# microsoft/maro

Hardware: AMD Instinct MI355X
Metric: env-steps/sec (decision events/sec), CIM global_trade.22p (higher is better)
Workload: dtype int32+f64

## Files before the change

maro_amd/csrc/cim_device.h:

```cpp
#pragma once
#include <math.h>
#include <stdint.h>

#include "cim_params.h"

#ifdef MRX_SPECIALIZED
#define KD(f) (MRXC_##f)
#define OD(f) (MRXC_obs_##f)
#define ODA(f, i) (MRXC_obs_##f(i))
#else
#define KD(f) (K.f)
#define OD(f) (O.f)
#define ODA(f, i) (O.f[i])
#endif

namespace cim {

#ifndef MRX_PROFILE_PHASES
struct Prof {
  MRX_DEV void mark(int) {}
  MRX_DEV void mark(int, long long) {}
  MRX_DEV void flush() {}
};
#endif
// ... 2133 lines not shown
#ifdef MRX_LEAN2
    const Tabs& T = L.tab;
    const int a_vs0 = wave::readlane(Z.s.vs0, v), a_Lr = a_vs0 & 63, a_rb = (int)((unsigned)a_vs0 >> 12), a_cb = wave::readlane(Z.s.vs2, v);
    const int a_lr = wave::lane() < a_Lr ? wave::lane() : 0;
    const int a_rp = T.route_port[a_rb + a_lr], a_rc = T.route_cidx[a_rb + a_lr], a_per = V_PERIOD(v);
#endif
    const int pe_v = FP(PA_EMPTY, p), ve_v = FV(VA_EMPTY, v), rs_v = FV(VA_REMAINING_SPACE, v), tc_v = FP(PA_TRANSFER_COST, p);
    const int pe = U(pe_v), ve = U(ve_v), rs = U(rs_v), tc = U(tc_v);
    int npe, nve;
    if (ty == 1) {
      if (q > ve) { c.status |= 1; continue; }
      npe = pe + q; nve = ve - q;
    } else {
      if (q > (pe < rs ? pe : rs)) { c.status |= 1; continue; }
      npe = pe - q; nve = ve + q;
    }
    FP(PA_EMPTY, p) = npe;
    FV(VA_EMPTY, v) = nve;
    FV(VA_REMAINING_SPACE, v) = rs - (nve - ve);
    c.opnum += q;
    FP(PA_TRANSFER_COST, p) = f_bits((float)((double)bits_f(tc) + (double)q));
    {
#ifdef MRX_LEAN2
      const uint64_t hit = wave::ballot(wave::lane() < a_Lr && a_rp == p);
      const int cc = hit ? a_cb + wave::readlane(a_rc, __builtin_ctzll(hit)) : -1;
      if (cc >= 0) { const int pl = U(L.frame[KD(f_plans) + cc]); L.frame[KD(f_plans) + cc] = pl + U(a_per); }
#else
      const int cc = plan_cell(L, v, p);
      if (cc >= 0) { const int pl = U(L.frame[KD(f_plans) + cc]); L.frame[KD(f_plans) + cc] = pl + U(V_PERIOD(v)); }
#endif
      else c.status |= 32;
    }
  }
  c.pend = consume_decisions(K, c.pend, L.priv[PH_CUR_VESSEL], c.n_answered);
  wave::sync();
}

template <bool PG, bool OBS>
MRX_DEV StepEnd body_run(const CimParams& K, const CimObs& O, int env, Lds& L, const StepIO& io, StepCtx& c, StepOut& out, Prof& prof, RingRegs& rr, Lean& Z) {
  const int lane = wave::lane();
  const int P = KD(P), V = KD(V);
  StepEnd end = {true, false, false};
  int t = c.t;
  bool fresh = c.fresh, finished = false;
  uint64_t pend = c.pend;
  int dec_v = -1;
  for (;;) {
    if (pend) {
      dec_v = __builtin_ctzll(pend);
      break;
    }
    if (!fresh) {
      if ((t + 1) % KD(resolution) == 0) {
        if (lane < P) FP(PA_ACC_FULFILLMENT, lane) = FP(PA_ACC_BOOKING, lane) - FP(PA_ACC_SHORTAGE, lane);
        wave::sync();
        take_snapshot(K, O, env, L, (t - KD(start_tick)) / KD(resolution));
        wave::sync();
        if (lane < P) { FP(PA_SHORTAGE, lane) = 0; FP(PA_BOOKING, lane) = 0; FP(PA_FULFILLMENT, lane) = 0; FP(PA_TRANSFER_COST, lane) = 0; }
        wave::sync();
      }
      if (t + 1 == KD(T)) {
        if ((t + 1) % KD(resolution) != 0) take_snapshot(K, O, env, L, (t - KD(start_tick)) / KD(resolution));
        finished = true;
        break;
      }
      t += 1;
    }
    prof.mark(PF_POST_STEP);
    fresh = false;
#ifdef MRX_LEAN2
    pend = run_tick_lean(K, env, L, t, c.pf, c.idx_buf, c.status, prof, end.buf_dirty, rr, Z);
#else
    pend = run_tick<PG>(K, env, L, t, c.pf, c.idx_ord, c.idx_buf, c.status, prof, end.ord_dirty, end.buf_dirty, rr);
#endif
    if (!pend && t + 1 < KD(T)) {
#ifdef MRX_LEAN2
      tick_prefetch_lean(K, env, L, t + 1, c.pf, Z);
#else
      tick_prefetch<PG>(K, env, L, t + 1, c.pf);
#endif
      tick_prefetch_land(c.pf);
    }
  }

  if (MRX_UNALIGNED_FRAMES && !finished) {
    const int fi0 = (t - KD(start_tick)) / KD(resolution), lo = KD(start_tick) + fi0 * KD(resolution);
    if (t > lo + (KD(resolution) - 1 - lo % KD(resolution))) {
      wave::sync();
      take_snapshot(K, O, env, L, fi0);
      wave::sync();
    }
  }
  long long acc_b = 0, acc_s = 0;
  if (lane < P) { acc_b = FP(PA_ACC_BOOKING, lane); acc_s = FP(PA_ACC_SHORTAGE, lane); }
  acc_b = wave::reduce_add(acc_b);
  acc_s = wave::reduce_add(acc_s);
  const int fi = (t - KD(start_tick)) / KD(resolution);
  out.kind = 1;
  if (KD(decision_mode) != 0) {
    int32_t* dec_out = io.dec_out;
    const uint64_t pm = finished ? 0ull : pend;
    const bool mine = lane < V && ((pm >> lane) & 1ull);
    if (mine) {
      const int r = __builtin_popcountll(pm & ((1ull << lane) - 1ull));
      const int v = lane, p = FV(VA_LOC_PORT_IDX, v);
      const int pe = FP(PA_EMPTY, p), rs = FV(VA_REMAINING_SPACE, v);
      int32_t* d = dec_out + 8 * r;
      d[0] = t; d[1] = p; d[2] = v; d[3] = pe < rs ? pe : rs; d[4] = FV(VA_EMPTY, v); d[5] = FV(VA_EARLY_DISCHARGE, v);
      d[6] = fi; d[7] = 1;
    }
    const int cnt = __builtin_popcountll(pm);
    if (lane < V && lane >= cnt) {
      int32_t* d = dec_out + 8 * lane;
      for (int j = 0; j < 8; j++) d[j] = 0;
      if (lane == 0) { d[0] = t; d[6] = fi; }
    }
  } else if (!finished) {
    {
      const int v = dec_v, p = FV(VA_LOC_PORT_IDX, v);
      const int pe = FP(PA_EMPTY, p), rs = FV(VA_REMAINING_SPACE, v);
      out.dec[0] = t; out.dec[1] = p; out.dec[2] = v;
      out.dec[3] = pe < rs ? pe : rs;
      out.dec[4] = FV(VA_EMPTY, v);
      out.dec[5] = FV(VA_EARLY_DISCHARGE, v);
      out.dec[6] = fi; out.dec[7] = 1;
    }
    if constexpr (OBS) {
      out.obs_on = true;
      const int tot = P * OD(np), npd = OD(np) > 0 ? OD(np) : 1;
#pragma unroll
      for (int j = 0; j < 8; j++) {
        const int i = lane + 64 * j;
        out.obs[j] = 0.0;
        if (i < tot) {
          const int p = i / npd, a = i - p * npd;
          const int attr = (int)((OD(pa_packed) >> (4 * a)) & 15u);
          out.obs[j] = port_attr_value(attr, FP(attr, p));
        }
      }
#pragma unroll
      for (int a = 0; a < 8; a++) out.vobs[a] = a < OD(nv) ? (double)FV(ODA(va, a), dec_v) : 0.0;
    }
  } else {
    out.dec[0] = t; out.dec[1] = 0; out.dec[2] = 0; out.dec[3] = 0; out.dec[4] = 0; out.dec[5] = 0;
    out.dec[6] = fi; out.dec[7] = 0;
  }
  out.met[0] = acc_b; out.met[1] = acc_s; out.met[2] = c.opnum;
  out.done = finished ? 1 : 0;
  out.tick = t;
  out.status = c.status;
  out.hint = (KD(decision_mode) == 0 && !MRX_UNALIGNED_FRAMES && (finished || (pend & ~(1ull << (dec_v & 63))))) ? 0 : 1;
  bool long_next = false;
  if (KD(start_tick) == 0 && !finished) {
#ifdef MRX_LEAN2
    const bool soon = lane < V && (vr_park(Z.w) ? Z.w.next : Z.w.evt) <= t + 1;
#else
    const bool soon = lane < V && (FV(VA_IS_PARKING, lane) ? V_NEXT(lane) : V_EVT(lane)) <= t + 1;
#endif
    long_next = wave::ballot(soon) == 0ull;
  }
  if (long_next && out.hint) out.hint = 2;
  if (lane == 0) {
    L.priv[PH_TICK] = t;
    L.priv[PH_FLAGS] = finished ? FL_FINISHED : (long_next ? FL_LONG : 0);
    L.priv[PH_PEND_LO] = (int32_t)(uint32_t)(pend & 0xffffffffull);
    L.priv[PH_PEND_HI] = (int32_t)(uint32_t)(pend >> 32);
    L.priv[PH_CUR_VESSEL] = dec_v;
    L.priv[PH_OPNUM_LO] = (int32_t)(uint32_t)((unsigned long long)c.opnum & 0xffffffffull);
    L.priv[PH_OPNUM_HI] = (int32_t)(c.opnum >> 32);
    L.priv[PH_IDX_ORDER] = c.idx_ord;
    L.priv[PH_IDX_BUFFER] = c.idx_buf;
    L.priv[PH_ACCB_LO] = (int32_t)(uint32_t)((unsigned long long)acc_b & 0xffffffffull); L.priv[PH_ACCB_HI] = (int32_t)(acc_b >> 32);
    L.priv[PH_ACCS_LO] = (int32_t)(uint32_t)((unsigned long long)acc_s & 0xffffffffull); L.priv[PH_ACCS_HI] = (int32_t)(acc_s >> 32);
  }
  wave::sync();
  prof.mark(PF_OUTPUT);
  return end;
}

template <bool OBS>
MRX_DEV void body_emit(const CimParams& K, const CimObs& O, int env, const StepIO& io, const StepOut& out, long long agent_seed) {
  const int lane = wave::lane();
  if (out.kind == 0) return;
  if (out.kind == 2) {
    if (lane < 8) io.dec_out[lane] = lane == 7 ? -1 : 0;
    if (lane < 3) io.met_out[lane] = 0;
    if (lane == 0) { *io.done_out = 1; if (O.agent_mode) agent_none(O, env); }
    return;
  }
  if (O.agent_mode && KD(decision_mode) == 0 && lane == 0) {
    if (out.dec[7] == 1 && !out.done) agent_answer(K, O, env, agent_seed, out.dec[0], out.dec[1], out.dec[2], out.dec[3], out.dec[4]);
    else agent_none(O, env);
  }
  if (KD(decision_mode) == 0) {
    if (lane == 0) {
#pragma unroll
      for (int j = 0; j < 8; j++) io.dec_out[j] = out.dec[j];
    }
    if constexpr (OBS) {
      if (out.obs_on) {
        const int tot = KD(P) * OD(np);
        double* op = O.ports + (size_t)env * tot;
#pragma unroll
        for (int j = 0; j < 8; j++) {
          const int i = lane + 64 * j;
          if (i < tot) op[i] = out.obs[j];
        }
#pragma unroll
        for (int a = 0; a < 8; a++)
          if (a < OD(nv) && lane == 0) O.vessel[(size_t)env * OD(nv) + a] = out.vobs[a];
      }
    }
  }
  if (lane == 0) {
    io.met_out[0] = out.met[0]; io.met_out[1] = out.met[1]; io.met_out[2] = out.met[2];
    *io.done_out = (uint8_t)out.done;
    K.tick[env] = out.tick;
    K.hint[env] = (uint8_t)out.hint;
    if (out.status) wave::global_or(&K.status[env], out.status);
  }
}

template <bool PG, bool OBS>
MRX_DEV StepEnd full_body(const CimParams& K, const CimObs& O, int env, Lds& L, const StepIO& io, int a0v, int a0p, int a0q, int a0t, Prof& prof, RingRegs& rr, Lean& Z) {
  StepCtx c;
  StepOut out;
  c.a0v = a0v; c.a0p = a0p; c.a0q = a0q; c.a0t = a0t;
  c.n_act = io.n_act; c.n_answered = io.n_answered;
  StepEnd end = {false, false, false};
  const long long agent_seed = O.agent_mode ? K.seed[env] : 0;
  if (body_open<PG>(K, env, L, c, out, Z)) {
    prof.mark(PF_LOAD);
    body_act(K, L, io.actions, c, Z);
    prof.mark(PF_ACTION);
    tick_prefetch_land(c.pf);
    prof.mark(PF_MT_LOAD);
    end = body_run<PG, OBS>(K, O, env, L, io, c, out, prof, rr, Z);
  }
  body_emit<OBS>(K, O, env, io, out, agent_seed);
  return end;
}

enum { PATH_PROBE = 0,
       PATH_FAST = 1,
       PATH_FULL = 2 };

template <bool PG, bool OBS>
MRX_DEV void step_env(const CimParams& K, const CimObs& O, int env, int32_t* lds, const StepIO& io, int path, int32_t* lds_ctab = nullptr) {
  Lds L = make_lds(K, lds);
  Prof prof;
  if (KD(decision_mode) == 0 && path != PATH_FULL) {
    FastRows rows;
    fast_rows_request<OBS>(K, O, env, rows);
    int hint = 0;
    if (path == PATH_PROBE) hint = K.hint[env];
    int f0v = 0, f0p = 0, f0q = 0, f0t = 0;
    if (io.actions) { f0v = io.actions[0]; f0p = io.actions[1]; f0q = io.actions[2]; f0t = io.actions[3]; }
    if (!U(hint) && fast_step<OBS>(K, O, env, rows, io.n_act > KD(max_actions) ? KD(max_actions) : io.n_act, f0v, f0p, f0q, f0t, io.dec_out,
                                   io.met_out, io.done_out)) {
#ifdef MRX_PROFILE_FAST_PATH
      prof.mark(13); prof.mark(14, 1);
      prof.flush();
#endif
      return;
    }
    prof.mark(12);
  }
  state_load_async<PG>(K, L, env);
  stage_tables(K, L, lds_ctab ? lds_ctab : lds + KD(l_ctab));
  RingRegs rr;
  ring_load(K, env, rr);
  Lean Z;
#ifdef MRX_LEAN2
  lean_stat_load(K, Z.s);
#endif
  int a0v = 0, a0p = 0, a0q = 0, a0t = 0;
  if (io.actions) { a0v = io.actions[0]; a0p = io.actions[1]; a0q = io.actions[2]; a0t = io.actions[3]; }
  wave::lds_dma_wait();
  const StepEnd e = full_body<PG, OBS>(K, O, env, L, io, a0v, a0p, a0q, a0t, prof, rr, Z);
  if (e.store) { state_store<PG>(K, L, env, e); ring_store(K, env, rr); }
  prof.mark(PF_STORE);
  prof.flush();
}

template <bool OBS>
MRX_DEV void fast_lanes_env(const CimParams& K, const CimObs& O, const StepBatch& B, const uint8_t* mask, int env) {
  if (env >= K.n_envs || (mask && !mask[env]) || K.hint[env]) return;
  const StepIO io = step_io(K, B, env);
  const int n_act = io.n_act > KD(max_actions) ? KD(max_actions) : io.n_act;
  if (KD(decision_mode) == 0 && fast_step_lane<OBS>(K, O, env, io.actions, n_act, io.dec_out, io.met_out, io.done_out)) return;
  K.order[wave::global_add(&K.sched[0], 1)] = env | MRX_ORDER_TICK;
}

template <bool PG, bool OBS>
MRX_DEV void step_loop(const CimParams& K, const CimObs& O, int32_t* lds, int w, int W, const StepBatch& B) {
  const int n_tick = U(wave::ld_uniform_v(K.sched + 0));
  for (int i = w; i < n_tick; i += W) {
    const int env = U(wave::ld_uniform_v(K.order + i)) & (MRX_ORDER_TICK - 1);
    step_env<PG, OBS>(K, O, env, lds, step_io(K, B, env), PATH_FULL);
    wave::sync();
  }
}

MRX_DEV int attr_slots(const CimParams& K, int node_type, int a) {
  if (node_type == 0) return 1;
  if (node_type == 1) {
    if (a == VA_PAST_STOP_LIST || a == VA_PAST_STOP_TICK_LIST) return KD(past_n);
    if (a == VA_FUTURE_STOP_LIST || a == VA_FUTURE_STOP_TICK_LIST) return KD(future_n);
    return 1;
  }
  return a == MA_FULL_ON_PORTS ? KD(P) * KD(P) : KD(V) * KD(P);
}

MRX_DEV int frame_word(const CimParams& K, int node_type, int a, int node, int s) {
  if (node_type == 0) return KD(f_ports) + a * KD(P) + node;
  if (node_type == 1) return KD(f_vessels) + a * KD(V) + node;
  if (a == MA_FULL_ON_PORTS) {
    const int k = K.pair_dense[s];
    return k < 0 ? -1 : KD(f_fop) + k;
  }
  const int c = K.cidx_dense[s];
  if (c < 0) return -1;
  return (a == MA_FULL_ON_VESSELS ? KD(f_fov) : KD(f_plans)) + c;
}

MRX_DEV int stop_list_value(const CimParams& K, int env, const int32_t* frame, int a, int v, int s) {
  const int Lr = K.v_route_len[v], rb = K.v_route_base[v], start = K.v_start[v];
  const uint32_t* srow = K.stops + ((size_t)env * KD(V) + v) * KD(SMAX);
  if (a == VA_PAST_STOP_LIST || a == VA_PAST_STOP_TICK_LIST) {
    const int j = frame[KD(f_vessels) + VA_NEXT_LOC_IDX * KD(V) + v] - KD(past_n) + s;
    if (j < 0) return -1;
    if (a == VA_PAST_STOP_LIST) return K.route_port[rb + (start + j) % Lr];
    if (j == 0) {
      const int32_t* hdr = K.priv + (size_t)env * KD(PW);
      const uint64_t zm = ((uint64_t)(uint32_t)hdr[PH_ZOMBIE_HI] << 32) | (uint32_t)hdr[PH_ZOMBIE_LO];
      if (!((zm >> v) & 1ull)) return 0;
    }
    return stop_arrival(srow[j < KD(SMAX) ? j : KD(SMAX) - 1]);
  }
  const int k = frame[KD(f_vessels) + VA_LAST_LOC_IDX * KD(V) + v];
  int tick = k == 0 ? 0 : stop_arrival(srow[k < KD(SMAX) ? k : KD(SMAX) - 1]);
  int x = (start + k) % Lr;
  const int lo = K.leg_off[v];
  for (int i = 0; i <= s; i++) {
    tick += K.leg_time[lo + x];
    x = (x + 1 == Lr) ? 0 : x + 1;
  }
  return a == VA_FUTURE_STOP_LIST ? K.route_port[rb + x] : tick;
}

MRX_DEV const int32_t* frame_of(const CimParams& K, int env, int fi) {
  const int s = (fi < 0 ? 0 : fi) % KD(S);
  const int32_t* hdr = K.priv + (size_t)env * KD(PW);
  const int flags = hdr[PH_FLAGS], tick = hdr[PH_TICK], held = K.ring_fi[(size_t)env * KD(S) + s];
  const bool paused = (flags & (FL_FRESH | FL_FINISHED)) == 0;
  const int cur_fi = (tick - KD(start_tick)) / KD(resolution);
  const int32_t* frame = nullptr;
  if (held == fi) frame = K.ring + ((size_t)env * KD(S) + s) * KD(FW);
  if (paused && s == cur_fi % KD(S)) frame = fi == cur_fi ? K.live + (size_t)env * KD(FW) : nullptr;
  return fi < 0 ? nullptr : frame;
}

MRX_DEV double query_elem(const CimParams& K, int node_type, const int32_t* ticks, int nt, int ticks_per_env,
                          const int32_t* nodes, int nn, int nodes_per_env, const int32_t* attrs, int na, long long row, int col) {
  const int ni = (int)(row % nn);
  const int ti = (int)((row / nn) % nt);
  const int env = (int)(row / ((long long)nn * nt));
  const int fi = ticks[(size_t)env * ticks_per_env + ti];
  const int32_t* frame = frame_of(K, env, fi);
  if (!frame) return 0.0;
  int a = 0, slot = col;
  for (int i = 0; i < na; i++) {
    const int ns = attr_slots(K, node_type, attrs[i]);
    if (slot < ns) { a = attrs[i]; break; }
    slot -= ns;
  }
  const int node = nodes[(size_t)env * nodes_per_env + ni];
  const int n_nodes = node_type == 0 ? KD(P) : node_type == 1 ? KD(V) : 1;
  if (node < 0 || node >= n_nodes) return 0.0;
  if (node_type == 1 && a >= VA_PAST_STOP_LIST) return (double)stop_list_value(K, env, frame, a, node, slot);
  const int w = frame_word(K, node_type, a, node, slot);
  if (w < 0) return a == MA_VESSEL_PLANS ? -1.0 : 0.0;
  const int32_t raw = frame[w];
  return (node_type == 0 && a == PA_TRANSFER_COST) ? (double)bits_f(raw) : (double)raw;
}

#undef FP
#undef FV
#undef FOPK
#undef FOVC
#undef PLANC
#undef V_EVT
#undef V_NEXT
#undef V_POS
#undef V_KRL
#undef V_PERIOD
#undef U
#undef RING_FULL
#undef RING_EMPTY

}
```

maro_amd/csrc/cim_step_kernels.h:

```cpp
extern "C" __global__ void __launch_bounds__(64)
mrx_k_cim_reset(CimParams K, const long long* __restrict__ seed_cmd, const uint8_t* __restrict__ mask, long long default_cmd) {
  extern __shared__ __attribute__((aligned(16))) int32_t lds[];
  const int env = blockIdx.x;
  if (mask && !mask[env]) return;
  cim::reset_env(K, env, lds, seed_cmd ? seed_cmd[env] : default_cmd);
}

extern "C" __global__ void __launch_bounds__(64)
mrx_k_cim_order_table(CimParams K, const long long* __restrict__ seed_cmd, const uint8_t* __restrict__ mask, long long default_cmd) {
  extern __shared__ __attribute__((aligned(16))) int32_t lds[];
  const int env = blockIdx.x;
  if (mask && !mask[env]) return;
  if ((seed_cmd ? seed_cmd[env] : default_cmd) == -1) return;
  cim::gen_order_table(K, env, lds);
}

#ifndef MRX_STEP_WAVES
#define MRX_STEP_WAVES 2
#endif
#ifdef MRX_SPECIALIZED
#define MRX_WG_WAVES MRXC_wg_waves
#else
#define MRX_WG_WAVES 1
#endif
#define MRX_STEP_KERNEL(NAME, PG, OBS, WAVES)                                                                            \
  extern "C" __global__ void __launch_bounds__(64 * MRX_WG_WAVES, WAVES)                                                 \
  NAME(CimParams K, CimObs O, cim::StepBatch B, const uint8_t* __restrict__ mask, int sorted) {                          \
    extern __shared__ __attribute__((aligned(16))) int32_t lds[];                                                       \
    const int w = MRX_WG_WAVES > 1 ? __builtin_amdgcn_readfirstlane((int)(threadIdx.x >> 6)) : 0;                        \
    const int slot = (int)blockIdx.x * MRX_WG_WAVES + w;                                                                \
    if (MRX_WG_WAVES > 1 && slot >= K.n_envs) return;                                                                   \
    int env = slot, path = cim::PATH_PROBE;                                                                             \
    if (sorted) {                                                                                                       \
      if (sorted == 2 && slot >= K.sched[0]) return;   \
      const int e = K.order[slot];                                                                                      \
      if (e < 0) return;                                                                                                \
      env = e & (MRX_ORDER_TICK - 1);                                                                                   \
      path = (e & MRX_ORDER_TICK) ? cim::PATH_FULL : cim::PATH_FAST;                                                    \
    } else if (mask && !mask[env]) {                                                                                    \
      return;                                                                                                           \
    }                                                                                                                   \
    cim::step_env<PG, OBS>(K, O, env, lds + w * KD(l_ctab), cim::step_io(K, B, env), path,                               \
                           lds + MRX_WG_WAVES * KD(l_ctab));                                                            \
  }
#ifdef MRX_SPECIALIZED
#define MRX_WANT(PG, OBS) ((PG) == (MRXC_pregen != 0) && (OBS) == ((MRXC_obs_np | MRXC_obs_nv) != 0))
#else
#define MRX_WANT(PG, OBS) 1
#endif
#define MRX_SPLIT_KERNELS(SUFFIX, PG, OBS, WAVES)                                                                       \
  extern "C" __global__ void __launch_bounds__(64)                                                                      \
  mrx_k_cim_fast_lanes##SUFFIX(CimParams K, CimObs O, cim::StepBatch B, const uint8_t* __restrict__ mask) {               \
    cim::fast_lanes_env<OBS>(K, O, B, mask, (int)(blockIdx.x * 64 + threadIdx.x));                                      \
  }                                                                                                                     \
  extern "C" __global__ void __launch_bounds__(64, WAVES)                                                               \
  mrx_k_cim_step_loop##SUFFIX(CimParams K, CimObs O, cim::StepBatch B) {                                                 \
    extern __shared__ __attribute__((aligned(16))) int32_t lds[];                                                       \
    cim::step_loop<PG, OBS>(K, O, lds, (int)blockIdx.x, (int)gridDim.x, B);                                             \
  }
#if MRX_WANT(0, 0)
MRX_STEP_KERNEL(mrx_k_cim_step, false, false, MRX_STEP_WAVES)
MRX_SPLIT_KERNELS(, false, false, MRX_STEP_WAVES)
#endif
#if MRX_WANT(0, 1)
MRX_STEP_KERNEL(mrx_k_cim_step_obs, false, true, MRX_STEP_WAVES)
MRX_SPLIT_KERNELS(_obs, false, true, MRX_STEP_WAVES)
#endif
#if MRX_WANT(1, 0)
MRX_STEP_KERNEL(mrx_k_cim_step_tab, true, false, MRX_STEP_WAVES)
MRX_SPLIT_KERNELS(_tab, true, false, MRX_STEP_WAVES)
#endif
#if MRX_WANT(1, 1)
MRX_STEP_KERNEL(mrx_k_cim_step_tab_obs, true, true, MRX_STEP_WAVES)
MRX_SPLIT_KERNELS(_tab_obs, true, true, MRX_STEP_WAVES)
#endif
#undef MRX_WANT
#undef MRX_STEP_KERNEL
#undef MRX_SPLIT_KERNELS
```

Measured before the change: 153.7 million.

## Add lane-parallel fast-path slots with ballot-driven full-step fallback in step kernel

Moves the per-slot dispatch into a new step_slot helper. Under MRX_LANE_WAVES with sorted==1, waves beyond the tick count each run the fast step for 64 environments at once, one per lane. Any lanes the fast path refuses are collected by ballot and then run serially through the full step_env on the same wave. This is meant to avoid a separate fast-lanes kernel launch and the one-env-per-wave cost of the fast path, at the price of serialised redo work and more branch complexity. Without the macro the behaviour is the same as before.

```diff
diff --git a/maro_amd/csrc/cim_device.h b/maro_amd/csrc/cim_device.h
--- a/maro_amd/csrc/cim_device.h
+++ b/maro_amd/csrc/cim_device.h
@@ -2459,6 +2459,70 @@
   }
 }
 
+template <bool PG, bool OBS>
+MRX_DEV void step_slot(const CimParams& K, const CimObs& O, const StepBatch& B, const uint8_t* mask, int sorted, int slot, int32_t* lds,
+                       int32_t* lds_ctab) {
+  int env = slot, path = PATH_PROBE;
+#ifdef MRX_LANE_WAVES
+  uint64_t redo = 0;
+  int redo_base = 0;
+  if (sorted == 1) {
+    const int e = K.order[slot], n_tick = K.sched[0], n_all = K.sched[1];
+    path = PATH_FULL;
+    if (e >= 0 && (e & MRX_ORDER_TICK)) {
+      env = e & (MRX_ORDER_TICK - 1);
+    } else {
+      const int w = slot - n_tick, n_fast = n_all - n_tick;
+      if (w < 0 || w >= ((n_fast + 63) >> 6)) return;
+      redo_base = n_tick + 64 * w;
+#ifdef MRX_PROFILE_FAST_PATH
+      Prof prof;
+#endif
+      const int i = redo_base + wave::lane();
+      bool refused = false;
+      if (i < n_all) {
+        const int lenv = K.order[i];
+        const StepIO io = step_io(K, B, lenv);
+        const int n_act = io.n_act > KD(max_actions) ? KD(max_actions) : io.n_act;
+        refused = !(KD(decision_mode) == 0 && fast_step_lane<OBS>(K, O, lenv, io.actions, n_act, io.dec_out, io.met_out, io.done_out));
+      }
+      redo = wave::ballot(refused);
+#ifdef MRX_PROFILE_FAST_PATH
+      prof.mark(13); prof.mark(14, __builtin_popcountll(wave::ballot(i < n_all) & ~redo));
+      prof.flush();
+#endif
+      if (!redo) return;
+      env = K.order[redo_base + __builtin_ctzll(redo)];
+      redo &= redo - 1;
+    }
+  } else
+#endif
+  if (sorted) {
+    if (sorted == 2 && slot >= K.sched[0]) return;
+    const int e = K.order[slot];
+    if (e < 0) return;
+    env = e & (MRX_ORDER_TICK - 1);
+    path = (e & MRX_ORDER_TICK) ? PATH_FULL : PATH_FAST;
+  } else if (mask && !mask[env]) {
+    return;
+  }
+#ifdef MRX_LANE_WAVES
+  for (;;) {
+    int z = 0;
+#if defined(__HIP_DEVICE_COMPILE__)
+    asm volatile("" : "+s"(z));
+#endif
+    step_env<PG, OBS>(K, O, env, lds + z, step_io(K, B, env), path, lds_ctab + z);
+    if (!redo) break;
+    wave::sync();
+    env = K.order[redo_base + __builtin_ctzll(redo)];
+    redo &= redo - 1;
+  }
+#else
+  step_env<PG, OBS>(K, O, env, lds, step_io(K, B, env), path, lds_ctab);
+#endif
+}
+
 MRX_DEV int attr_slots(const CimParams& K, int node_type, int a) {
   if (node_type == 0) return 1;
   if (node_type == 1) {
diff --git a/maro_amd/csrc/cim_step_kernels.h b/maro_amd/csrc/cim_step_kernels.h
--- a/maro_amd/csrc/cim_step_kernels.h
+++ b/maro_amd/csrc/cim_step_kernels.h
@@ -30,18 +30,7 @@
     const int w = MRX_WG_WAVES > 1 ? __builtin_amdgcn_readfirstlane((int)(threadIdx.x >> 6)) : 0;                        \
     const int slot = (int)blockIdx.x * MRX_WG_WAVES + w;                                                                \
     if (MRX_WG_WAVES > 1 && slot >= K.n_envs) return;                                                                   \
-    int env = slot, path = cim::PATH_PROBE;                                                                             \
-    if (sorted) {                                                                                                       \
-      if (sorted == 2 && slot >= K.sched[0]) return;   \
-      const int e = K.order[slot];                                                                                      \
-      if (e < 0) return;                                                                                                \
-      env = e & (MRX_ORDER_TICK - 1);                                                                                   \
-      path = (e & MRX_ORDER_TICK) ? cim::PATH_FULL : cim::PATH_FAST;                                                    \
-    } else if (mask && !mask[env]) {                                                                                    \
-      return;                                                                                                           \
-    }                                                                                                                   \
-    cim::step_env<PG, OBS>(K, O, env, lds + w * KD(l_ctab), cim::step_io(K, B, env), path,                               \
-                           lds + MRX_WG_WAVES * KD(l_ctab));                                                            \
+    cim::step_slot<PG, OBS>(K, O, B, mask, sorted, slot, lds + w * KD(l_ctab), lds + MRX_WG_WAVES * KD(l_ctab));             \
   }
 #ifdef MRX_SPECIALIZED
 #define MRX_WANT(PG, OBS) ((PG) == (MRXC_pregen != 0) && (OBS) == ((MRXC_obs_np | MRXC_obs_nv) != 0))
```

Result: faster. 276.7 million (median of 6 runs) (+80.0%).
